# EternityJune25/ComoRAG

Measured on AMD Instinct MI355X. Metric: top-k queries/sec, higher is better.
Workload: dtype bf16; 1 GPU; brute-force top-20 over 10000000 x 768 bf16 rows, batch 64, row-sharded over 1 GPU(s) (north_star target config); rows=10000000, dim=768, batch=64, k=20, query_batches_rotated=4, device=AMD Radeon Graphics (gfx950:sramecc+:xnack-), n_cu=256, repeats=1, exchange=none (1 shard)

## Files before the change

### comorag_amd/csrc/api.hip

```cpp
#include <hip/hip_runtime.h>

#include <algorithm>
#include <cmath>
#include <cstdarg>
#include <cstdio>
#include <cstdlib>
#include <cstring>
#include <chrono>
#include <atomic>
#include <climits>
#include <map>
#include <memory>
#include <mutex>
#include <shared_mutex>
#include <string>
#include <vector>

#include "../../include/comorag_hip.h"
#include "cmr_kernels.h"
#include "cmr_internal.h"
#include "index_state.h"
#include "search_plan.h"
#include "prefilter_host.h"

// ... 30 lines not shown
#define CMR_STR_(x) #x
#define CMR_STR(x) CMR_STR_(x)
#define OPT_FIELD(f) [](cmr_index* i, long long v) { i->f = (decltype(i->f))v; }
#define OPT_READ(expr) [](const cmr_index* i) -> long long { return expr; }
const Option kOptions[] = {
    {"scan_ring", OPT_FIELD(force_ring), Option::any, 0, 0, 0, nullptr, nullptr},
    {"scan_asm_ring", OPT_FIELD(force_asm), Option::any, 0, 0, 0, nullptr, nullptr},
    {"scan_grid", OPT_FIELD(force_grid), Option::any, 0, 0, 0, nullptr, nullptr},
    {"scan_no_sample", OPT_FIELD(no_sample), Option::any, 0, 0, 0, nullptr, nullptr},
    {"scan_no_wide", OPT_FIELD(no_wide), Option::any, 0, 0, 0, nullptr, nullptr},
    {"scan_no_tiny", OPT_FIELD(no_tiny), Option::any, 0, 0, 0, nullptr, nullptr},
    {"scan_no_small", OPT_FIELD(no_small), Option::any, 0, 0, 0, nullptr, nullptr},
    {"small_max_panels", OPT_FIELD(small_max_panels), Option::clamp, 32, 6144, 0, nullptr, nullptr},
    {"tiny_multi", OPT_FIELD(tiny_multi), Option::any, 0, 0, 0, nullptr, nullptr},
    {"zero_copy", OPT_FIELD(zero_copy), Option::any, 0, 0, 0, nullptr, nullptr},
    {"sample_single", OPT_FIELD(single_level), Option::any, 0, 0, 0, nullptr, nullptr},
    {"sample_single_max", OPT_FIELD(single_level_max), Option::clamp, 0, LLONG_MAX, 0, nullptr, nullptr},
    {"sample_tau_in_scan", OPT_FIELD(tau_in_scan), Option::any, 0, 0, 0, nullptr, nullptr},
    {"scan_fin", OPT_FIELD(scan_fin), Option::any, 0, 0, 0, nullptr, nullptr},
    {"sync_poll", OPT_FIELD(sync_poll), Option::any, 0, 0, 0, nullptr, nullptr},
    {"scan_fin_dense", OPT_FIELD(fin_dense), Option::clamp, 1, 1 << 16, 0, nullptr, nullptr},
    {"scan_fin_cap", OPT_FIELD(fin_cap), Option::oneof, 0, 128, 256, "scan_fin_cap must be 0, 128 or 256", nullptr},
    {"scan_fin_suppliers", OPT_FIELD(fin_suppliers), Option::clamp, 0, CMR_FIN_SLOTS / CMR_SCAN_WAVES, 0, nullptr, nullptr},
    {"scan_fin_spin", OPT_FIELD(fin_spin), Option::clamp, 0, 1000, 0, nullptr, nullptr},
    {"scan_fin_queries", OPT_FIELD(fin_max_q), Option::clamp, 1, CMR_FIN_MAX_QUERIES, 0, nullptr, nullptr},
    {"sample_div", OPT_FIELD(sample_div), Option::clamp, 2, LLONG_MAX, 0, nullptr, nullptr},
    {"sample_maxmul", OPT_FIELD(sample_maxmul), Option::clamp, 0, LLONG_MAX, 0, nullptr, nullptr},
    {"pipe_reserve_cus", OPT_FIELD(reserve_cus), Option::any, 0, 0, 0, nullptr, nullptr},
    {"pipe_slots", OPT_FIELD(pipe_slots), Option::any, 0, 0, 0, nullptr, nullptr},
    {"wide_mode", OPT_FIELD(wide_mode), Option::range, 0, 2, 0, "wide_mode must be 0 (default), 1 (register-resident kernel) or 2 (query-split grid)", nullptr},
    {"stream_nt", OPT_FIELD(stream_nt), Option::any, 0, 0, 0, nullptr, nullptr},
    {"pipe_dual_scan", OPT_FIELD(dual_scan), Option::any, 0, 0, 0, nullptr, nullptr},
    {"pipe_cu_mask", OPT_FIELD(cu_mask), Option::any, 0, 0, 0, nullptr, nullptr},
    {"exact_cand", OPT_FIELD(exact_cand), Option::range, 2, CMR_MAX_K, 0, "exact_cand must be in [2, " CMR_STR(CMR_MAX_K) "]", OPT_READ(i->exact_cand)},
    {"combine", [](cmr_index* i, long long v) { i->combine.store((int)v, std::memory_order_relaxed); }, Option::zero_or, 2, cmr_combine::kMaxWidth, 0,
     "combine must be 0 (off) or in [2, " CMR_STR(CMR_PPR_MAX_BATCH) "]", OPT_READ(i->combine.load(std::memory_order_relaxed))},
    {"combine_wait_us", [](cmr_index* i, long long v) { i->combine_wait_us.store(v, std::memory_order_relaxed); }, Option::clamp, 0, 10000000, 0, nullptr,
     OPT_READ(i->combine_wait_us.load(std::memory_order_relaxed))},
    {"prefilter", OPT_FIELD(prefilter), Option::range, -1, 2, 0, "prefilter must be -1 (auto), 0 (off), 1 (on) or 2 (on, the filter keeps every row)", OPT_READ(i->prefilter)},
    {"prefilter_rescore_wgs", OPT_FIELD(pf_rescore_wgs), Option::clamp, 0, 1024, 0, nullptr, nullptr},
    {"prefilter_tighten", OPT_FIELD(pf_tighten), Option::range, 0, 1, 0, "prefilter_tighten must be 0 or 1", OPT_READ(i->pf_tighten)},
    {"prefilter_pair_cap", OPT_FIELD(pf_pair_cap), Option::clamp, 0, 1 << 20, 0, nullptr, OPT_READ(i->pf_pair_cap)},
    {"prefilter_wave_cap", OPT_FIELD(pf_wave_cap), Option::clamp, 0, 1 << 20, 0, nullptr, OPT_READ(i->pf_wave_cap)},
    {"prefilter_sample", OPT_FIELD(pf_sample), Option::range, -1, 1, 0, "prefilter_sample must be -1 (auto), 0 (bf16 sampling) or 1 (int8 sample)", OPT_READ(i->pf_sample)},
    {"prefilter_sample_panels", OPT_FIELD(pf_sample_panels), Option::clamp, 0, INT_MAX, 0, nullptr, OPT_READ(i->pf_sample_panels)},
    {"prefilter_sample_run", OPT_FIELD(pf_sample_run), Option::clamp, 0, 1 << 16, 0, nullptr, OPT_READ(i->pf_sample_run)},
    {"prefilter_sample_wave_cap", OPT_FIELD(pf_sample_wave_cap), Option::clamp, 0, 1 << 20, 0, nullptr, OPT_READ(i->pf_sample_wave_cap)},
    {"prefilter_sample_level0", OPT_FIELD(pf_sample_level0), Option::clamp, 0, 128, 0, nullptr, OPT_READ(i->pf_sample_level0)},
    {"prefilter_sample_active", nullptr, Option::any, 0, 0, 0, nullptr, OPT_READ(i->prefilter_sample_active)},
    {"prefilter_sample_pairs", nullptr, Option::any, 0, 0, 0, nullptr, OPT_READ(q8_read_counter(i, Q8Counter::sample_pairs))},
    {"prefilter_sample_overflow", nullptr, Option::any, 0, 0, 0, nullptr, OPT_READ(q8_read_counter(i, Q8Counter::sample_overflow))},
    {"prefilter_active", nullptr, Option::any, 0, 0, 0, nullptr, OPT_READ(i->prefilter_active)},
    {"prefilter_rows", nullptr, Option::any, 0, 0, 0, nullptr, OPT_READ(i->q8c.q8 ? i->q8c.rows : 0)},
    {"prefilter_bytes", nullptr, Option::any, 0, 0, 0, nullptr, OPT_READ((long long)i->q8c.bytes(i->dpad))},
    {"prefilter_candidates", nullptr, Option::any, 0, 0, 0, nullptr, OPT_READ(q8_read_counter(i, Q8Counter::candidates))},
    {"prefilter_pairs", nullptr, Option::any, 0, 0, 0, nullptr, OPT_READ(q8_read_counter(i, Q8Counter::pairs))},
    {"prefilter_pair_overflow", nullptr, Option::any, 0, 0, 0, nullptr, OPT_READ(q8_read_counter(i, Q8Counter::pair_overflow))},
    {"prefilter_wave_overflow", nullptr, Option::any, 0, 0, 0, nullptr, OPT_READ(q8_read_counter(i, Q8Counter::wave_overflow))},
    {"last_route", nullptr, Option::any, 0, 0, 0, nullptr, OPT_READ(i->last_route.load(std::memory_order_relaxed))},
    {"pipe_dual_scan_active", nullptr, Option::any, 0, 0, 0, nullptr, OPT_READ(i->dual_active)},
    {"pipe_dual_scan_wide_active", nullptr, Option::any, 0, 0, 0, nullptr, OPT_READ(i->dual_wide_active)},
    {"pipe_cu_mask_active", nullptr, Option::any, 0, 0, 0, nullptr, OPT_READ(i->pipe.last_masked)},
    {"pipe_scan_cus", nullptr, Option::any, 0, 0, 0, nullptr, OPT_READ(i->pipe.last_masked ? i->pipe.scan_cus : i->n_cu)},
    {"combine_batches", nullptr, Option::any, 0, 0, 0, nullptr, OPT_READ(i->combiner.batches())},
    {"combine_queries", nullptr, Option::any, 0, 0, 0, nullptr, OPT_READ(i->combiner.queries())},
    {"combine_max_width", nullptr, Option::any, 0, 0, 0, nullptr, OPT_READ(i->combiner.max_width())},
};
#undef OPT_FIELD
#undef OPT_READ

const Option* find_option(const char* name) {
    for (const Option& o : kOptions) if (strcmp(o.name, name) == 0) return &o;
    return nullptr;
}

int set_option(cmr_index* idx, const char* name, long long v) {
    const Option* o = find_option(name ? name : "");
    if (!o || !o->store) return fail(CMR_ERR_INVALID, "unknown option '%s'", name ? name : "");
    const bool refused = o->kind == Option::oneof ? (v != o->a && v != o->b && v != o->c) : o->kind == Option::range ? (v < o->a || v > o->b) : o->kind == Option::zero_or ? (v != 0 && (v < o->a || v > o->b)) : false;
    if (refused) return fail(CMR_ERR_INVALID, "%s", o->reject);
    if (o->kind == Option::clamp) v = std::max(o->a, std::min(v, o->b));
    o->store(idx, v);
    return CMR_OK;
}

int remap_ids_enqueue(cmr_index* idx, int64_t* ids_dev, long long n, hipStream_t s);
long long to_local_row(const cmr_index* idx, long long gid) {
    if (gid < 0) return -1;
    if (idx->single_block()) { const long long r = gid - idx->id_base; return (r >= 0 && r < idx->n) ? r : -1; }
    const size_t nb = idx->blk_local.size();
    size_t b = std::upper_bound(idx->blk_global.begin(), idx->blk_global.end(), gid) - idx->blk_global.begin();
    if (b == 0) return -1;
    --b;
    const long long len = (b + 1 < nb ? idx->blk_local[b + 1] : idx->n) - idx->blk_local[b];
    const long long off = gid - idx->blk_global[b];
    return off < len ? idx->blk_local[b] + off : -1;
// ... 186 lines not shown
        a.fin = (int*)ws->fin_ctl.p; a.fin_pmax = (u64*)ws->fin_pmax.p; a.fin_tau = (u64*)ws->fin_tau.p; a.fin_dense = (u64*)ws->fin_dense.p;
        a.fin_first = p.fin_first; a.fin_wgs = p.fin_wgs; a.fin_mul = p.fin_mul; a.fin_dcap = p.fin_dcap; a.fin_spin = p.fin_spin;
        a.out_ids = ids_dev; a.out_scores = scores_dev; a.out_min = min_dev; a.out_max = max_dev; a.id_base = kernel_id_base(idx);
        fin_state = (const int*)ws->fin_ctl.p + CMR_FIN_STATE;
        if (ws->done_ptr && idx->single_block()) a.fin_done = ws->done_ptr;
    }
    if (p.prefilter) { if ((rc = q8_filter(idx, f, a, sm))) return rc; }
    else HIP_TRY(p.wide ? cmr_launch_scan_wide(g, a, sm) : p.fin ? cmr_launch_scan_fin(g, a, sm) : p.masked ? cmr_launch_scan_masked(g, a, sm) : cmr_launch_scan_topk(g, a, sm));
    if (prof) {
        HIP_TRY(hipEventRecord(pe.b, sm));
        std::lock_guard<std::mutex> pg(idx->prof_mu);
        idx->prof_events.push_back(pe);
        idx->prof_bytes = p.prefilter ? prefilter_bytes(idx, p) : algorithmic_bytes(idx, nqp, k);
    }
    if (a.fin_done) {
        ws->lazy.due = true;
        ws->lazy.lists = (const u64*)ws->lists.p; ws->lazy.cnt = (const int*)ws->cnt.p; ws->lazy.W = p.W; ws->lazy.NQ = p.NQ; ws->lazy.cap = g.cap; ws->lazy.nqp = nqp; ws->lazy.k = k;
        ws->lazy.mm = (const float2*)ws->mm.p; ws->lazy.id_base = kernel_id_base(idx); ws->lazy.ids = ids_dev; ws->lazy.scores = scores_dev; ws->lazy.mn = min_dev; ws->lazy.mx = max_dev;
        ws->lazy.state = fin_state;
        ws->done_used = true;
        return CMR_OK;
    }
    if (sq != sm) {
        HIP_TRY(hipEventRecord(st.ev_scan, sm));
        HIP_TRY(hipStreamWaitEvent(sq, st.ev_scan, 0));
    }
    if (p.prefilter && (rc = q8_rescore(f, sq))) return rc;
    HIP_TRY(cmr_launch_merge_query((const u64*)ws->lists.p, (const int*)ws->cnt.p, p.W, p.NQ, g.cap, nqp, k, (const float2*)ws->mm.p,
                                   kernel_id_base(idx), ids_dev, scores_dev, min_dev, max_dev, nullptr, sq, G > 1, fin_state));
    return remap_ids_enqueue(idx, ids_dev, (long long)nqp * k, sq);
}

int plan_and_enqueue_pass(cmr_index* idx, Workspace* ws, const PassStreams& st, const PassSplit& ps, int k, int reserve_cus, const float* q_dev,
                          const float* min_score, int64_t* ids_dev, float* scores_dev, float* min_dev, float* max_dev, int prefilter = 0) {
    PassPlan plan;
    PassRequest rq = st.request(ps.nqp, k, ps.route, min_score != nullptr, reserve_cus);
    rq.prefilter = prefilter;
    int rc = plan_pass(idx, rq, &plan);
    if (rc) return rc;
    if (ps.q0 == 0)
        idx->last_route.store(route_code(plan, min_score != nullptr) | (ps.nqp < ps.nq ? CMR_ROUTE_MORE_PASSES : 0), std::memory_order_relaxed);
    return enqueue_pass(idx, ws, st, plan, q_dev + (size_t)ps.q0 * idx->dim, min_score, ids_dev + (size_t)ps.q0 * k, scores_dev + (size_t)ps.q0 * k,
                        min_dev ? min_dev + ps.q0 : nullptr, max_dev ? max_dev + ps.q0 : nullptr);
}

int search_enqueue(cmr_index* idx, Workspace* ws, const float* q_dev, int nq, int k, int64_t* ids_dev, float* scores_dev,
                   float* min_dev, float* max_dev, const float* min_score = nullptr) {
    if (k > CMR_MAX_K) {
        if (min_score) return fail(CMR_ERR_UNSUPPORTED, "threshold search supports k <= %d", CMR_MAX_K);
        return search_large_k_enqueue(idx, ws, q_dev, nq, k, ids_dev, scores_dev, min_dev, max_dev);
    }
    if (const int kind = small_path_kind(idx, nq, k, min_score != nullptr)) {
        const long long npanels = idx->npanels();
        idx->last_route.store(route_code(kind == 1 ? CMR_ROUTE_TINY : CMR_ROUTE_SMALL), std::memory_order_relaxed);
        { int rc_ = arm_flag(ws, ws->stream); if (rc_) return rc_; }
        HIP_TRY(ws->d_out.ensure(cmr_tiny_scratch_bytes(nq, (int)npanels, k, idx->tiny_multi, idx->small_max_panels)));
        if (!ws->arrive.p) {
            HIP_TRY(ws->arrive.ensure(sizeof(int)));
            HIP_TRY(hipMemsetAsync(ws->arrive.p, 0, sizeof(int), ws->stream));
        }
        HIP_TRY(cmr_launch_tiny_search(idx->dtype, idx->corpus, q_dev, nq, idx->dim, idx->dpad, idx->n, k, kernel_id_base(idx), ws->d_out.p,
                                       ids_dev, scores_dev, min_dev, max_dev, ws->flag_ptr, idx->tiny_multi ? (int*)ws->arrive.p : nullptr, idx->small_max_panels, ws->stream,
                                       (ws->done_ptr && idx->single_block()) ? ws->done_ptr : nullptr));
        if (ws->done_ptr && idx->single_block()) ws->done_used = true;
        return remap_ids_enqueue(idx, ids_dev, (long long)nq * k, ws->stream);
    }
    const PassStreams st = PassStreams::one(ws->stream);
    for (PassSplit ps(idx, nq); ps.next();) {
        int rc = plan_and_enqueue_pass(idx, ws, st, ps, k, 0, q_dev, min_score, ids_dev, scores_dev, min_dev, max_dev);
        if (rc) return rc;
// ... 59 lines not shown
    Pipe T;
    auto undo = [&]() {
        T.destroy_streams();
        for (auto& slot : ev) for (hipEvent_t& e : slot) if (e) { (void)hipEventDestroy(e); e = nullptr; }
        T.scan_cus = T.wide_cus = 0;
    };
    int rc = create_pipe_streams(idx, T, mask, idx->dual_scan < 0 ? mask != 0 : idx->dual_scan != 0);
    if (rc && mask) {
        undo();
        mask = 0;
        rc = create_pipe_streams(idx, T, 0, idx->dual_scan > 0);
    }
    if (rc) { undo(); return rc; }
    auto make_events = [&]() -> int {
        for (auto& slot : ev) for (hipEvent_t& e : slot) HIP_TRY(hipEventCreateWithFlags(&e, hipEventDisableTiming));
        return CMR_OK;
    };
    rc = make_events();
    if (rc) { undo(); return rc; }
    for (int i = 0; i < Pipe::n_streams; ++i) if (i != Pipe::sq) P.st[i] = T.st[i];
    P.scan_cus = T.scan_cus; P.wide_cus = T.wide_cus;
    for (int i = 0; i < CMR_PIPE_SLOTS; ++i) {
        P.slot[i].pre_done = ev[i][0]; P.slot[i].main_done = ev[i][1]; P.slot[i].scan_done = ev[i][2];
        P.slot[i].ws.stream = P.st[Pipe::sm];
    }
    P.st[Pipe::sq] = T.st[Pipe::sq];
    return CMR_OK;
}

int search_pipelined_enqueue_locked(cmr_index* idx, const float* q_dev, int nq, int k, int64_t* ids_dev, float* scores_dev, float* min_dev,
                                    float* max_dev, hipEvent_t wait_event, hipEvent_t* done_event, const float* min_score, bool may_prefilter = false) {
    Pipe& P = idx->pipe;
    { int rc_ = ensure_pipe(idx); if (rc_) return rc_; }
    P.nslots = std::min(CMR_PIPE_SLOTS, std::max(2, idx->pipe_slots));
    if (k > CMR_MAX_K) return fail(CMR_ERR_UNSUPPORTED, "pipelined search supports k <= %d", CMR_MAX_K);
    const bool masked = P.scan_cus != 0 && (idx->cu_mask > 0 || idx->short_scan());
    const bool twins = P.scan_cus != 0 && !masked;
    P.last_masked = masked ? 1 : 0;
    hipStream_t const nsp = P.st[twins ? Pipe::usp : Pipe::sp], wsp = P.st[twins ? Pipe::uwp : Pipe::wp];
    PassSplit ps(idx, nq);
    if (wait_event) {
        HIP_TRY(hipStreamWaitEvent(nsp, wait_event, 0));
        if (ps.any_wide()) HIP_TRY(hipStreamWaitEvent(wsp, wait_event, 0));
    }
    int prefilter = prefilter_eligible(idx, min_score != nullptr, min_dev || max_dev, nq, may_prefilter);
    if (prefilter && !q8_ensure_companion(idx, nsp)) prefilter = 0;
    idx->prefilter_active = 0;
    idx->prefilter_sample_active = 0;
    PipeSlot* last = nullptr;
    while (ps.next()) {
        const bool wide = ps.wide_streams();
        PipeSlot* sl = &P.slot[P.next++ % (unsigned)P.nslots];
        hipStream_t sp = wide ? wsp : nsp;
        if (sl->used) {
            HIP_TRY(hipStreamWaitEvent(sp, sl->scan_done, 0));
        }
        const bool dual = !twins && P.st[wide ? Pipe::wm2 : Pipe::sm2] != nullptr && (idx->dual_scan > 0 || idx->short_scan());
        if (!wide) idx->dual_active = dual ? 1 : 0;
        else idx->dual_wide_active = dual ? 1 : 0;
        hipStream_t sm = P.st[twins ? (wide ? Pipe::uwm : Pipe::usm)
                                    : wide ? ((dual && (P.nwscan++ & 1)) ? Pipe::wm2 : Pipe::wm) : ((dual && (P.nscan++ & 1)) ? Pipe::sm2 : Pipe::sm)];
        const PassStreams st{sp, sm, P.st[Pipe::sq], sl->pre_done, sl->scan_done, sl->used ? sl->main_done : nullptr};
        int rc = plan_and_enqueue_pass(idx, &sl->ws, st, ps, k, (masked && !wide) ? idx->n_cu - P.scan_cus : (masked && wide) ? idx->n_cu - P.wide_cus : idx->reserve_cus,
                                       q_dev, min_score, ids_dev, scores_dev, min_dev, max_dev, wide ? 0 : prefilter);
        if (rc) return rc;
        HIP_TRY(hipEventRecord(sl->main_done, P.st[Pipe::sq]));
        sl->used = true;
        last = sl;
    }
    if (done_event) *done_event = last ? last->main_done : nullptr;
    return CMR_OK;
}
int search_pipelined_enqueue(cmr_index* idx, const float* q_dev, int nq, int k, int64_t* ids_dev, float* scores_dev, float* min_dev,
                             float* max_dev, hipEvent_t wait_event, hipEvent_t* done_event, const float* min_score = nullptr, bool may_prefilter = false) {
    std::lock_guard<std::mutex> pl(idx->pipe_mu);
    return search_pipelined_enqueue_locked(idx, q_dev, nq, k, ids_dev, scores_dev, min_dev, max_dev, wait_event, done_event, min_score, may_prefilter);
}

int scores_enqueue(cmr_index* idx, Workspace* ws, const float* q_dev, int nq, float* out_dev, long long ld) {
    hipStream_t s = ws->stream;
    CmrScanGeom g{};
    const int per_pass = idx->narrow_width(nq);
    const long long npanels = idx->npanels();
    { int rc_ = arm_flag(ws, s); if (rc_) return rc_; }
    for (int q0 = 0; q0 < nq; q0 += per_pass) {
        const int nqp = std::min(per_pass, nq - q0);
        int rc = make_geom(idx, nqp, 1, false, &g);
        if (rc) return rc;
        HIP_TRY(ws->qfrag.ensure((size_t)g.nqt * g.ks * 1024));
        HIP_TRY(cmr_launch_prep_queries(idx->dtype, q_dev + (size_t)q0 * idx->dim, nqp, idx->dim, idx->dpad, g.nqt, ws->qfrag.p,
                                        ws->flag_ptr, s));
        CmrScanArgs a{};
        a.corpus = idx->corpus; a.qfrag = ws->qfrag.p; a.nrows = idx->n; a.npanels = (int)npanels; a.k = 1;
        a.scores = out_dev + (size_t)q0 * ld; a.ld = ld; a.nq = nqp;
        HIP_TRY(cmr_launch_scan_scores(g, a, s));
    }
    return CMR_OK;
// ... 466 lines not shown
        idx->blk_retired.clear();
    }
    idx->d_blk = d;
    idx->blk_local.assign(local_start, local_start + n_blocks);
    idx->blk_global.assign(global_start, global_start + n_blocks);
    idx->id_base = global_start[0];
    return CMR_OK;
}

int32_t cmr_index_set_option(cmr_index_t* idx, const char* name, int64_t value) {
    if (!idx || !name) return fail(CMR_ERR_INVALID, "NULL argument");
    std::unique_lock<std::shared_mutex> lk(idx->mu);
    return set_option(idx, name, value);
}

int32_t cmr_index_get_option(cmr_index_t* idx, const char* name, int64_t* value) {
    if (!idx || !name || !value) return fail(CMR_ERR_INVALID, "NULL argument");
    std::shared_lock<std::shared_mutex> lk(idx->mu);
    const Option* o = find_option(name);
    if (!o || !o->read) return fail(CMR_ERR_INVALID, "unknown readable option '%s'", name);
    *value = o->read(idx);
    return CMR_OK;
}

int32_t cmr_index_pipeline_stream(cmr_index_t* idx, int32_t which, void** stream) {
    if (!idx || !stream) return fail(CMR_ERR_INVALID, "NULL argument");
    if (which < 0 || which > 2) return fail(CMR_ERR_INVALID, "which must be 0 (pre), 1 (scan) or 2 (post)");
    int rc = cmr_set_device(idx->device);
    if (rc) return rc;
    std::lock_guard<std::mutex> pl(idx->pipe_mu);
    Pipe& P = idx->pipe;
    rc = ensure_pipe(idx);
    if (rc) return rc;
    const bool twins = P.scan_cus != 0 && !P.last_masked && P.next != 0;
    *stream = (void*)P.st[which == 0 ? (twins ? Pipe::usp : Pipe::sp) : which == 1 ? (twins ? Pipe::usm : Pipe::sm) : Pipe::sq];
    return CMR_OK;
}

int32_t cmr_index_query_status(cmr_index_t* idx, int32_t* nonfinite) {
    if (!idx || !nonfinite) return fail(CMR_ERR_INVALID, "NULL argument");
    *nonfinite = 0;
    std::shared_lock<std::shared_mutex> lk(idx->mu);
    int rc = cmr_set_device(idx->device);
    if (rc) return rc;
    std::vector<Workspace*> wss;
    {
        std::lock_guard<std::mutex> pl(idx->pipe_mu);
        for (int i = 0; i < CMR_PIPE_SLOTS; ++i) if (idx->pipe.slot[i].used) wss.push_back(&idx->pipe.slot[i].ws);
        if (idx->pipe.st[Pipe::sq]) {
            for (hipStream_t st : idx->pipe.st) if (st) HIP_TRY(hipStreamSynchronize(st));
        }
    }
    {
        std::lock_guard<std::mutex> g(idx->ws_mu);
        for (auto& kv : idx->stream_ws) wss.push_back(kv.second);
    }
    for (Workspace* ws : wss) {
        if (!ws->flag_ptr) continue;
        if (ws->stream || !ws->own_stream) HIP_TRY(hipStreamSynchronize(ws->stream));
        int h = 0;
        HIP_TRY(hipMemcpy(&h, ws->flag_ptr, sizeof(int), hipMemcpyDeviceToHost));
        if (h) {
            *nonfinite = 1;
            HIP_TRY(hipMemset(ws->flag_ptr, 0, sizeof(int)));
        }
    }
    return CMR_OK;
}
// ... 696 lines not shown
```

### comorag_amd/csrc/index_state.h

```cpp
#pragma once
#include <hip/hip_runtime.h>

#include <algorithm>
#include <atomic>
#include <cstring>
#include <map>
#include <mutex>
#include <shared_mutex>
#include <vector>

#include "../../include/comorag_hip.h"
#include "cmr_kernels.h"
#include "cmr_internal.h"
#include "combine.h"

#define CMR_DT_F32 0
#define CMR_PANEL_ROWS 32
#define CMR_SCAN_WAVES 8
#define CMR_CORPUS_SLACK (128 * 1024)

namespace {

int elem_size(int dtype) { return dtype == CMR_F32 ? 4 : 2; }
int round_up(int x, int m) { return (x + m - 1) / m * m; }
// ... 51 lines not shown
        if (h_pin) { hipError_t e = hipHostFree(h_pin); if (e != hipSuccess) return e; h_pin = nullptr; h_pin_dev = nullptr; h_pin_cap = 0; }
        const size_t want = std::max(need, h_pin_cap * 2);
        hipError_t e = hipHostMalloc(&h_pin, want, hipHostMallocDefault);
        if (e != hipSuccess) return e;
        e = hipHostGetDevicePointer(&h_pin_dev, h_pin, 0);
        if (e != hipSuccess) { (void)hipHostFree(h_pin); h_pin = nullptr; return e; }
        h_pin_cap = want;
        return hipSuccess;
    }
    void release() {
        qfrag.release(); lists.release(); cnt.release(); mm.release(); flag.release(); tau.release();
        s_lists.release(); s_cnt.release(); s_mm.release(); arrive.release();
        fin_ctl.release(); fin_pmax.release(); fin_tau.release(); fin_dense.release(); fin_mm.release();
        d_q.release(); d_ids.release(); d_scores.release(); d_min.release(); d_max.release(); d_cand.release(); d_out.release();
        d_mask.release();
        d_pack.release();
        q8.release();
        x.release();
        if (h_pin) (void)hipHostFree(h_pin);
        h_pin = nullptr; h_pin_dev = nullptr; h_pin_cap = 0;
        if (own_stream && stream) (void)hipStreamDestroy(stream);
    }
};

struct ProfEvent { hipEvent_t a, b; };

constexpr size_t kMappedAppendMax = 128 * 1024;
constexpr size_t kZeroCopyMax = 256 * 1024;

struct PipeSlot { Workspace ws; hipEvent_t pre_done = nullptr, scan_done = nullptr, main_done = nullptr; bool used = false; };
#define CMR_PIPE_SLOTS 4
struct Pipe {
    enum Stream { sp, sm, sm2, wp, wm, wm2, usp, usm, uwp, uwm, sq, n_streams };
    hipStream_t st[n_streams] = {};
    PipeSlot slot[CMR_PIPE_SLOTS]; unsigned next = 0; int nslots = 2; unsigned nscan = 0, nwscan = 0; int scan_cus = 0, wide_cus = 0; int last_masked = 0;
    void destroy_streams() { for (hipStream_t& s : st) if (s) { (void)hipStreamDestroy(s); s = nullptr; } }
};

}

struct cmr_index {
    int device = 0;
    int dim = 0, dpad = 0, dtype = 0;
    uint32_t flags = 0;
    int n_cu = 256;
    long long n = 0;
    long long cap_panels = 0;
    void* corpus = nullptr;
    float* shadow = nullptr;
    std::shared_mutex mu;
    std::mutex ws_mu;
    std::vector<Workspace*> free_ws;
    std::map<hipStream_t, Workspace*> stream_ws;
    DevBuf stage;
    void* h_pin = nullptr;
    void* h_pin_dev = nullptr;
    size_t h_pin_cap = 0;
    int* d_flag = nullptr;
    std::mutex prof_mu;
    bool prof_on = false;
    int prof_every = 1;
    unsigned prof_seq = 0;
    std::vector<ProfEvent> prof_events;
    double prof_bytes = 0.0;
    int force_ring = 0;
    int force_asm = -1;
    int force_grid = 0;
    int no_sample = 0;
// ... 10 lines not shown
    int stream_nt = -1;
    int wide_mode = 0;
    int tau_in_scan = 1;
    int sync_poll = 1;
    int scan_fin = 1;
    int fin_dense = 16384;
    int fin_cap = 0;
    int fin_suppliers = 0;
    int fin_spin = 0;
    int fin_max_q = 8;
    int dual_wide_active = 0;
    std::atomic<long long> last_route{0};
    int dual_active = 0;
    std::atomic<int> combine{0};
    std::atomic<long long> combine_wait_us{0};
    cmr_combine::Combiner combiner;
    long long id_base = 0;
    std::vector<long long> blk_local, blk_global;
    long long* d_blk = nullptr;
    std::vector<void*> blk_retired;
    int sample_maxmul = 0;
    int sample_div = 32;
    int prefilter = -1;
    int pf_rescore_wgs = 0;
    int pf_tighten = 1;
    int pf_pair_cap = 16384;
    int pf_wave_cap = 0;
    int pf_sample = -1;
    int pf_sample_panels = 0;
    int pf_sample_run = 0;
    int pf_sample_wave_cap = 0;
    int pf_sample_level0 = 0;
    int prefilter_sample_active = 0;
    Q8Companion q8c;
    int prefilter_active = 0;
    Q8LastPass q8_last;
    int pipe_slots = 3;
    int reserve_cus = -1;
    std::mutex pipe_mu;
    Pipe pipe;
    float* d_stats = nullptr;
    int exact_cand = CMR_MAX_K;
    ExactScratch x_slot[CMR_PIPE_SLOTS];
    unsigned x_next = 0;

    size_t panel_bytes() const { return (size_t)CMR_PANEL_ROWS * dpad * elem_size(dtype); }
    long long npanels() const { return panels_of(n); }
    int ks() const { return dtype == CMR_F32 ? dpad / 8 : dpad / 16; }
    int narrow_max() const { return cmr_scan_max_nqt(dtype, dpad) >= 2 ? 64 : 32; }
    int narrow_width(int nq) const { return nq > 32 ? narrow_max() : 32; }
    double scan_us() const { return (double)npanels() * panel_bytes() / 6.0e6; }
    bool short_scan() const { return scan_us() < 1000.0; }
    bool single_block() const { return blk_local.size() <= 1; }
    bool small_operands_fit() const { return (size_t)ks() * 1024 <= 143 * 1024; }
};

namespace {

long long kernel_id_base(const cmr_index* idx) { return idx->single_block() ? idx->id_base : 0; }

Workspace* acquire_ws(cmr_index* idx, hipStream_t user_stream, bool dev_api) {
    std::lock_guard<std::mutex> g(idx->ws_mu);
    if (dev_api && user_stream) {
        auto it = idx->stream_ws.find(user_stream);
        if (it != idx->stream_ws.end()) return it->second;
        Workspace* w = new Workspace();
        w->stream = user_stream;
        idx->stream_ws[user_stream] = w;
        return w;
    }
// ... 65 lines not shown
```

### comorag_amd/csrc/search_plan.h

```cpp
#pragma once
#include <numeric>

#include "index_state.h"

bool cmr_ring_audit_ok(int dtype, int nqt, int cap, int ring, int mode);
static const long long kMaxMergeLists = 4096;
constexpr bool kPrefilterSampleAuto = false;
static const long long kQ8SamplePanels = 8192;
static const int kQ8SampleRun = 16;
static const int kQ8SampleLevel0 = 64;

namespace {

int make_geom(const cmr_index* idx, int nq, int k, bool topk, CmrScanGeom* g) {
    const int max_nqt = cmr_scan_max_nqt(idx->dtype, idx->dpad);
    if (max_nqt == 0) return cmr_fail(CMR_ERR_UNSUPPORTED, "dim %d too large for the LDS-resident query tile (dtype %d)", idx->dim, idx->dtype);
    g->dtype = idx->dtype;
    g->dpad = idx->dpad;
    g->nqt = (nq > 32 && max_nqt >= 2) ? 2 : 1;
    g->cap = (topk && k > 32) ? 256 : 128;
    const int ks = idx->ks();
    g->ring = (ks % 16 == 0) ? 16 : 8;
    if (idx->force_ring == 8 || (idx->force_ring == 16 && ks % 16 == 0)) g->ring = idx->force_ring;
    const int mode = topk ? 0 : 1;
    g->asm_ring = cmr_ring_audit_ok(g->dtype, g->nqt, g->cap, g->ring, mode) ? 1 : 0;
    if (idx->force_asm == 0) g->asm_ring = 0;
    if (idx->force_asm == 1 && !cmr_ring_audit_ok(g->dtype, g->nqt, g->cap, g->ring, mode))
        return cmr_fail(CMR_ERR_UNSUPPORTED, "CMR_SCAN_ASM_RING=1 but variant (dtype %d nqt %d cap %d ring %d) failed the ISA audit", g->dtype, g->nqt, g->cap, g->ring);
    if (!cmr_scan_geom(g)) return cmr_fail(CMR_ERR_UNSUPPORTED, "scan geometry does not fit LDS (dpad %d nqt %d)", idx->dpad, g->nqt);
    const int bpc = g->lds <= 80 * 1024 ? 2 : 1;
    long long grid = (idx->npanels() + CMR_SCAN_WAVES - 1) / CMR_SCAN_WAVES;
    grid = std::min<long long>(grid, (long long)idx->n_cu * bpc);
    if (idx->force_grid > 0) grid = std::min<long long>(grid, idx->force_grid);
    g->grid = (int)std::max<long long>(grid, 1);
    return CMR_OK;
}

double algorithmic_bytes(const cmr_index* idx, int nq, int k) {
    return (double)idx->npanels() * CMR_PANEL_ROWS * idx->dpad * elem_size(idx->dtype) + (double)nq * idx->dim * 4 + (double)nq * k * 12;
}

int balanced_grid(long long npanels, int grid, int lists_per_wg) {
    int best = grid;
    double best_cost = -1.0;
    for (int g = grid; g >= std::max(1, grid - grid / 8); --g) {
        const long long W = (long long)g * lists_per_wg;
        const double cost = (double)((npanels + W - 1) / W * W) * (1.0 + 0.0005 * (grid - g));
        if (best_cost < 0 || cost < best_cost) { best_cost = cost; best = g; }
    }
    return best;
}


enum class Route { narrow, wide, quad };

struct PassRequest {
    int nqp = 0, k = 0;
    Route route = Route::narrow;
    bool has_min_score = false;
    bool single_stream = false;
    bool pipelined = false;
    int reserve_cus = 0;
    int prefilter = 0;
    bool masked = false;
};

struct PassPlan {
    int nqp = 0, k = 0;
    bool wide = false;
    CmrScanGeom g{};
    bool fin = false;
    bool masked = false;
    int prefilter = 0;
    int rescore_grid = 0;
    int pair_cap = 0;
    int wave_cap = 0;
    bool sample_q8 = false;
    int s_run = 0, s_stride = 0, s_nruns = 0, s_wave_cap = 0, s_pair_cap = 0;
    int G = 1;
    int n_levels = 0;
    struct Level { long long panels; int grid, Wl, clog, stride; } level[2] = {};
    bool single_level = false;
    bool tau_in_scan = false;
    int reserve_cus = 0;
    int lists_per_wg = CMR_SCAN_WAVES;
    int NQ = 0, W = 0, Ws = 0, tiles = 0, NQA = 0;
    int fin_first = 0, fin_wgs = 0, fin_mul = 1, fin_dcap = 0, fin_spin = 0;
    struct { size_t qfrag, lists, cnt, mm, s_lists, s_cnt, s_mm, tau, fin_ctl, fin_pmax, fin_tau, fin_mm, fin_dense, q8[Q8_NBUF]; } bytes = {};
};

int plan_pass(const cmr_index* idx, const PassRequest& rq, PassPlan* out) {
    PassPlan& p = *out;
    p = PassPlan{};
    const int nqp = rq.nqp, k = rq.k;
    const bool wide = rq.route == Route::wide, quad = rq.route == Route::quad;
    p.nqp = nqp; p.k = k; p.wide = wide;
    if (rq.masked && (wide || quad || rq.prefilter)) return cmr_fail(CMR_ERR_INVALID, "a filtered pass is a narrow pass without the pre-filter");
    p.masked = rq.masked;
    CmrScanGeom& g = p.g;
    const long long npanels = idx->npanels();
    int rc = make_geom(idx, quad ? std::min(nqp, idx->narrow_max()) : nqp, k, true, &g);
    if (rc) return rc;
    const int G = quad ? (nqp + g.nqt * 32 - 1) / (g.nqt * 32) : 1;
    p.G = G;
    g.stream_default_policy = idx->stream_nt < 0 ? (G > 1 ? 1 : 0) : (idx->stream_nt ? 0 : 1);
    const int lists_per_wg = wide ? 1 : CMR_SCAN_WAVES;
// ... 14 lines not shown
    p.fin = fin;
    const bool prefilter = rq.prefilter && !wide && G == 1 && !fin;
    const bool sample_q8 = prefilter && rq.prefilter == 1 && idx->pf_tighten && idx->pf_pair_cap > 0 && npanels >= 4096 &&
                           (idx->pf_sample < 0 ? kPrefilterSampleAuto : idx->pf_sample == 1);
    long long level_panels[2] = {0, 0};
    long long bf16_level1 = 0;
    int n_levels = 0;
    bool single_level = false;
    if (!idx->no_sample && npanels >= 256 && !rq.has_min_score && !fin) {
        const long long s0 = sample_q8 ? std::max<long long>(idx->pf_sample_level0 > 0 ? idx->pf_sample_level0 : kQ8SampleLevel0, k) : std::max<long long>(16, k);
        single_level = !wide && !prefilter && idx->single_level && k <= 32 && nqp <= 8 && npanels >= 4096 && (long long)nqp * npanels <= idx->single_level_max;
        level_panels[n_levels++] = single_level ? 128 : s0;
        if (npanels >= 4096 && !single_level) {
            const long long maxmul = idx->sample_maxmul > 0 ? idx->sample_maxmul : (wide ? 512 : prefilter ? kMaxMergeLists : 128);
            const long long b0 = std::max<long long>(16, k);
            long long s1 = std::min<long long>(std::max<long long>(npanels / idx->sample_div, 8 * b0), maxmul * b0);
            if (!wide) s1 = std::min<long long>(s1, kMaxMergeLists);
            if (s1 < npanels / 2) bf16_level1 = s1;
            if (sample_q8) {
                level_panels[n_levels++] = idx->pf_sample_panels > 0 ? std::min<long long>(idx->pf_sample_panels, npanels)
                                                                     : std::min<long long>(std::max<long long>(npanels / idx->sample_div, 8 * s0), kQ8SamplePanels);
            } else if (bf16_level1) level_panels[n_levels++] = bf16_level1;
        }
    }
    p.n_levels = n_levels;
    p.single_level = single_level;
    p.sample_q8 = sample_q8 && n_levels == 2;
    const long long max_sample = std::max(level_panels[0], p.sample_q8 ? 0 : level_panels[1]);
    int reserve_cus = rq.reserve_cus;
    if (reserve_cus < 0) {
        if (!max_sample) reserve_cus = 0;
        else if (wide) {
            reserve_cus = 32;
        } else if (prefilter && idx->scan_us() >= 1250.0) {
            reserve_cus = 32;
        } else {
            const long long rounds = (long long)((0.7 * idx->scan_us() - 200.0) / 200.0);
            const long long wgs = std::max<long long>(1, (max_sample + lists_per_wg - 1) / lists_per_wg) * G;
            reserve_cus = rounds >= 1 ? (int)std::min<long long>(64, std::max<long long>(8, (wgs + rounds - 1) / rounds)) : 64;
        }
    }
    p.reserve_cus = reserve_cus;
    auto sample_grid = [&](long long spn) -> int {
        if (!wide) return (int)((spn + lists_per_wg - 1) / lists_per_wg);
        const int cap_wgs = rq.pipelined && reserve_cus > 0 ? reserve_cus : idx->n_cu;
        return (int)std::min<long long>(spn, std::max<long long>(cap_wgs, (spn + 47) / 48));
    };
    const int Ws = max_sample ? std::max(sample_grid(level_panels[0]), n_levels > 1 && !p.sample_q8 ? sample_grid(level_panels[1]) : 0) * lists_per_wg : 0;
    int NQ, W, tiles;
    if (wide) {
        const int nqb = cmr_wide_queries(idx->dtype, idx->dpad);
        g.nqt = 1;
        g.grid = (int)std::max<long long>(1, std::min<long long>(npanels, idx->n_cu));
        if (reserve_cus > 0 && g.grid > idx->n_cu / 2) g.grid = std::max(g.grid - reserve_cus, idx->n_cu / 2);
        NQ = nqb; W = g.grid; tiles = nqb / 32;
    } else if (G > 1) {
        if (reserve_cus > 0 && g.grid > idx->n_cu / 2) g.grid = std::max(g.grid - reserve_cus, idx->n_cu / 2);
        int vg = g.grid / G;
        if (vg >= 8) vg &= ~7;
        g.grid = std::max(vg, 1);
        NQ = g.nqt * 32; W = g.grid * CMR_SCAN_WAVES; tiles = G * g.nqt;
    } else {
        if (reserve_cus > 0 && g.grid > idx->n_cu / 2) g.grid = std::max(g.grid - reserve_cus, idx->n_cu / 2);
        if (!idx->force_grid) g.grid = balanced_grid(npanels, g.grid, CMR_SCAN_WAVES);
        NQ = g.nqt * 32; W = g.grid * CMR_SCAN_WAVES; tiles = g.nqt;
    }
    if (prefilter) {
        p.prefilter = rq.prefilter;
        p.rescore_grid = idx->pf_rescore_wgs > 0 ? idx->pf_rescore_wgs : std::min(idx->n_cu, 1024);
        W = p.rescore_grid * cmr_q8_rescore_waves();
        p.pair_cap = (rq.prefilter == 1 && idx->pf_tighten) ? idx->pf_pair_cap : 0;
        p.bytes.q8[Q8_QPACK] = (size_t)2 * tiles * (idx->dpad / 32) * 1024;
        p.bytes.q8[Q8_QCONST] = (size_t)NQ * sizeof(float4);
        p.bytes.q8[Q8_CAND] = (size_t)idx->cap_panels * CMR_PANEL_ROWS * sizeof(unsigned);
        p.bytes.q8[Q8_NCAND] = sizeof(unsigned);
        const long long fw = (long long)g.grid * CMR_SCAN_WAVES;
        p.wave_cap = !p.pair_cap ? 0 : idx->pf_wave_cap > 0 ? idx->pf_wave_cap : (int)std::min<long long>(1 << 20, (((long long)NQ * p.pair_cap + fw - 1) / fw + 63) / 64 * 64);
        p.bytes.q8[Q8_WREC] = std::max<size_t>((size_t)fw * p.wave_cap * 16, 16);
        p.bytes.q8[Q8_WCNT] = (size_t)fw * sizeof(unsigned);
        p.bytes.q8[Q8_PAIR] = std::max<size_t>((size_t)NQ * p.pair_cap * 16, 16);
        p.bytes.q8[Q8_PAIRCNT] = (size_t)NQ * sizeof(unsigned);
        p.bytes.q8[Q8_KEEP] = (size_t)idx->cap_panels * sizeof(unsigned);
        p.bytes.q8[Q8_TAU] = (size_t)NQ * sizeof(float);
        if (p.sample_q8) {
            const long long s1 = level_panels[1];
            const long long run = std::min<long long>(idx->pf_sample_run > 0 ? idx->pf_sample_run : kQ8SampleRun, s1);
            long long nruns = (s1 + run - 1) / run, stride = npanels / nruns;
            if (stride < run) { stride = run; nruns = std::min(nruns, (npanels + run - 1) / run); }
            p.s_run = (int)run; p.s_stride = (int)stride; p.s_nruns = (int)nruns;
            p.s_wave_cap = idx->pf_sample_wave_cap > 0 ? idx->pf_sample_wave_cap : (int)std::min<long long>(1 << 20, (run * CMR_PANEL_ROWS * NQ / 16 + 63) / 64 * 64);
            p.s_pair_cap = p.pair_cap;
            const long long sw = (nruns + CMR_SCAN_WAVES - 1) / CMR_SCAN_WAVES * CMR_SCAN_WAVES;
            p.bytes.q8[Q8_SWREC] = (size_t)sw * p.s_wave_cap * 16;
            p.bytes.q8[Q8_SWCNT] = (size_t)sw * sizeof(unsigned);
            p.bytes.q8[Q8_SPAIR] = (size_t)NQ * p.s_pair_cap * 16;
            p.bytes.q8[Q8_SPAIRCNT] = (size_t)NQ * sizeof(unsigned);
        }
    }
    const int NQA = G * NQ;
    p.NQ = NQ; p.W = W; p.Ws = Ws; p.tiles = tiles; p.NQA = NQA;
    p.bytes.qfrag = (size_t)tiles * g.ks * 1024;
// ... 14 lines not shown
        }
        L.grid = sample_grid(spn);
        L.Wl = L.grid * lists_per_wg;
        L.grid *= G;
        L.clog = spn >= 64 ? 3 : 0;
        const long long nchunks = (spn + (1 << L.clog) - 1) >> L.clog;
        L.stride = (int)(npanels / nchunks);
    }
    p.tau_in_scan = n_levels > 0 && single_level && idx->tau_in_scan && NQ == 32 && nqp <= 2 && k <= 64 && !p.prefilter;
    if (G > 1) g.grid *= G;
    if (fin) {
        p.fin_dcap = idx->fin_dense;
        p.fin_spin = idx->fin_spin;
        p.bytes.fin_ctl = CMR_FIN_CTL * sizeof(int);
        p.bytes.fin_pmax = (size_t)32 * CMR_FIN_SLOTS * 8;
        p.bytes.fin_tau = 32 * 8;
        p.bytes.fin_mm = (size_t)32 * 512 * 8;
        p.bytes.fin_dense = (size_t)32 * p.fin_dcap * 8;
        p.fin_first = std::min(g.grid, idx->n_cu);
        p.fin_wgs = std::min(std::min(idx->fin_suppliers > 0 ? idx->fin_suppliers : (npanels >= 131072 ? 128 : 64), CMR_FIN_SLOTS / CMR_SCAN_WAVES), p.fin_first);
        p.fin_mul = 1;
        for (int m = std::max(1, (int)(g.grid * 0.6180339887)); m < g.grid; ++m)
            if (std::gcd(m, g.grid) == 1) { p.fin_mul = m; break; }
    }
    return CMR_OK;
}

long long route_code(int path, int n_levels = 0, bool tau_in_scan = false, bool single_level = false, int nqt = 1, bool threshold = false) {
    return (long long)path | ((long long)n_levels << 4) | ((long long)(tau_in_scan ? 1 : 0) << 6) | ((long long)(single_level ? 1 : 0) << 7) | ((long long)nqt << 8) |
           ((long long)(threshold ? 1 : 0) << 10);
}
long long route_code(const PassPlan& p, bool threshold) {
    const int path = p.wide ? CMR_ROUTE_WIDE : p.G > 1 ? CMR_ROUTE_QUERY_SPLIT : p.fin ? CMR_ROUTE_FIN : CMR_ROUTE_CHAIN;
    return route_code(path, p.n_levels, p.tau_in_scan, p.single_level, p.g.nqt, threshold) | (p.masked ? CMR_ROUTE_FILTERED : 0);
}


bool wide_pass_is_quad(const cmr_index* idx) {
    if (idx->wide_mode == 2) return true;
    if (idx->wide_mode == 1) return false;
    return cmr_wide_queries(idx->dtype, idx->dpad) == 0;
}
bool short_two_tile_pass(const cmr_index* idx, int left) {
    if (idx->wide_mode != 0 || idx->no_wide || cmr_wide_queries(idx->dtype, idx->dpad) == 0) return false;
    if (cmr_scan_max_nqt(idx->dtype, idx->dpad) < 2 || left <= 64 || left > 128) return false;
    return idx->short_scan();
}
int wide_pass_queries(const cmr_index* idx) {
    if (idx->no_wide) return 0;
    if (!wide_pass_is_quad(idx)) return cmr_wide_queries(idx->dtype, idx->dpad);
    return 4 * idx->narrow_max();
}

struct PassSplit {
    const cmr_index* idx;
    const int nq, narrow, wideq;
    const bool quad;
    int q0 = 0, nqp = 0;
    Route route = Route::narrow;
    PassSplit(const cmr_index* i, int nq_) : idx(i), nq(nq_), narrow(i->narrow_width(nq_)), wideq(wide_pass_queries(i)), quad(wide_pass_is_quad(i)) {}
    bool any_wide() const { return wideq > 0 && nq > narrow; }
    bool wide_streams() const { return route != Route::narrow; }
    bool next() {
        q0 += nqp;
        if (q0 >= nq) return false;
        const int left = nq - q0;
        const bool wide = wideq > 0 && left > narrow;
// ... 16 lines not shown
```

### include/comorag_hip.h

```cpp
#ifndef COMORAG_HIP_H
#define COMORAG_HIP_H

#include <stdint.h>

#ifdef __cplusplus
extern "C" {
#endif

#define CMR_ABI_VERSION 2

enum cmr_status {
    CMR_OK = 0,
    CMR_ERR_INVALID = -1,
    CMR_ERR_NO_DEVICE = -2,
    CMR_ERR_HIP = -3,
    CMR_ERR_OOM = -4,
    CMR_ERR_NONFINITE = -5,
    CMR_ERR_UNSUPPORTED = -6
};

enum cmr_dtype { CMR_F32 = 0, CMR_BF16 = 1, CMR_F16 = 2 };

#define CMR_FLAG_KEEP_F32 1u

// ... 17 lines not shown

int32_t cmr_index_append(cmr_index_t* idx, const float* rows_f32, int64_t n);
int32_t cmr_index_append_dev(cmr_index_t* idx, const float* rows_f32_dev, int64_t n, void* stream);

int32_t cmr_index_search(cmr_index_t* idx, const float* q_f32, int32_t nq, int32_t k,
                         int64_t* out_ids, float* out_scores, float* out_min, float* out_max);
int32_t cmr_index_search_min_score(cmr_index_t* idx, const float* q_f32, int32_t nq, int32_t k, float min_score,
                                   int64_t* out_ids, float* out_scores);
int32_t cmr_index_search_min_score_dev(cmr_index_t* idx, const float* q_f32_dev, int32_t nq, int32_t k, float min_score,
                                       int64_t* out_ids_dev, float* out_scores_dev, void* stream);
int32_t cmr_index_search_min_score_pipelined(cmr_index_t* idx, const float* q_f32_dev, int32_t nq, int32_t k, float min_score,
                                             int64_t* out_ids_dev, float* out_scores_dev, void* wait_event, void** done_event);
int32_t cmr_index_search_dev(cmr_index_t* idx, const float* q_f32_dev, int32_t nq, int32_t k,
                             int64_t* out_ids_dev, float* out_scores_dev, float* out_min_dev,
                             float* out_max_dev, void* stream);

int32_t cmr_index_search_masked(cmr_index_t* idx, const float* q_f32, int32_t nq, int32_t k,
                                const uint32_t* allow_words, int64_t n_words,
                                int64_t* out_ids, float* out_scores, float* out_min, float* out_max);
int32_t cmr_index_search_masked_dev(cmr_index_t* idx, const float* q_f32_dev, int32_t nq, int32_t k,
                                    const uint32_t* allow_words_dev, int64_t n_words,
                                    int64_t* out_ids_dev, float* out_scores_dev,
                                    float* out_min_dev, float* out_max_dev, void* stream);

int32_t cmr_index_search_pipelined(cmr_index_t* idx, const float* q_f32_dev, int32_t nq, int32_t k,
                                   int64_t* out_ids_dev, float* out_scores_dev, float* out_min_dev,
                                   float* out_max_dev, void* wait_event, void** done_event);

int32_t cmr_index_set_id_base(cmr_index_t* idx, int64_t base);
int32_t cmr_index_set_id_blocks(cmr_index_t* idx, int32_t n_blocks, const int64_t* local_start, const int64_t* global_start);
int32_t cmr_index_set_option(cmr_index_t* idx, const char* name, int64_t value);
#define CMR_ROUTE_MORE_PASSES (1 << 11)
#define CMR_ROUTE_FILTERED (1 << 12)
#define CMR_ROUTE_TINY 1
#define CMR_ROUTE_SMALL 2
#define CMR_ROUTE_CHAIN 3
#define CMR_ROUTE_FIN 4
#define CMR_ROUTE_WIDE 5
#define CMR_ROUTE_QUERY_SPLIT 6
#define CMR_ROUTE_LARGE_K 7
#define CMR_ROUTE_SCORES_SINGLE 8
#define CMR_ROUTE_SCORES 9
#define CMR_ROUTE_SORTED 10
int32_t cmr_index_get_option(cmr_index_t* idx, const char* name, int64_t* value);
int32_t cmr_index_pipeline_stream(cmr_index_t* idx, int32_t which, void** stream);

int32_t cmr_index_query_status(cmr_index_t* idx, int32_t* nonfinite);

int32_t cmr_stream_wait_event(void* stream, void* event);
int32_t cmr_event_synchronize(void* event);

int32_t cmr_index_scores(cmr_index_t* idx, const float* q_f32, int32_t nq, float* out, int64_t ld);
int32_t cmr_index_scores_dev(cmr_index_t* idx, const float* q_f32_dev, int32_t nq, float* out_dev,
                             int64_t ld, void* stream);

int32_t cmr_index_sorted_scores(cmr_index_t* idx, const float* q_f32, int32_t nq, int64_t* out_ids,
                                float* out_scores, float* out_min, float* out_max);

int32_t cmr_index_rescore(cmr_index_t* idx, const float* q_f32, int32_t nq, const int64_t* cand,
                          int32_t n_cand, int32_t k, int64_t* out_ids, float* out_scores);

int32_t cmr_index_search_exact(cmr_index_t* idx, const float* q_f32, int32_t nq, int32_t k, int64_t* out_ids, float* out_scores,
                               int32_t* out_exact);
int32_t cmr_index_search_exact_pipelined(cmr_index_t* idx, const float* q_f32_dev, int32_t nq, int32_t k, int64_t* ids_dev,
                                         float* scores_dev, int32_t* exact_dev, void* wait_event, void** done_event);
int32_t cmr_index_round_stats(cmr_index_t* idx, float* max_row_norm, float* max_round_err);
// ... 136 lines not shown
```

Baseline: 41760 queries/s.

## Route prefiltered narrow passes onto CU-masked wide stream set with dual scan streams

Adds a 'filter' pipeline stream set that sends prefiltered narrow passes through the CU-masked wide-stream pair (wp/wm/wm2). On long scans it can alternate between two scan streams, reserving the non-wide CUs for the prefilter and rescore work. The set is picked automatically when the prefilter is active, the scan is long and the batch is wider than 32 queries. Slot count becomes set-dependent: 2 for the filter set and 3 otherwise. This aims to overlap prefilter and scan stages better, at the cost of fewer slots and a different CU partition.

```diff
diff --git a/comorag_amd/csrc/api.hip b/comorag_amd/csrc/api.hip
--- a/comorag_amd/csrc/api.hip
+++ b/comorag_amd/csrc/api.hip
@@ -86,6 +86,8 @@
     {"stream_nt", OPT_FIELD(stream_nt), Option::any, 0, 0, 0, nullptr, nullptr},
     {"pipe_dual_scan", OPT_FIELD(dual_scan), Option::any, 0, 0, 0, nullptr, nullptr},
     {"pipe_cu_mask", OPT_FIELD(cu_mask), Option::any, 0, 0, 0, nullptr, nullptr},
+    {"pipe_prefilter_dual", OPT_FIELD(pf_dual), Option::range, -1, 1, 0, "pipe_prefilter_dual must be -1 (auto), 0 (off) or 1 (on)", OPT_READ(i->pf_dual)},
+    {"pipe_prefilter_dual_active", nullptr, Option::any, 0, 0, 0, nullptr, OPT_READ(i->pf_dual_active)},
     {"exact_cand", OPT_FIELD(exact_cand), Option::range, 2, CMR_MAX_K, 0, "exact_cand must be in [2, " CMR_STR(CMR_MAX_K) "]", OPT_READ(i->exact_cand)},
     {"combine", [](cmr_index* i, long long v) { i->combine.store((int)v, std::memory_order_relaxed); }, Option::zero_or, 2, cmr_combine::kMaxWidth, 0,
      "combine must be 0 (off) or in [2, " CMR_STR(CMR_PPR_MAX_BATCH) "]", OPT_READ(i->combine.load(std::memory_order_relaxed))},
@@ -115,7 +117,7 @@
     {"pipe_dual_scan_active", nullptr, Option::any, 0, 0, 0, nullptr, OPT_READ(i->dual_active)},
     {"pipe_dual_scan_wide_active", nullptr, Option::any, 0, 0, 0, nullptr, OPT_READ(i->dual_wide_active)},
     {"pipe_cu_mask_active", nullptr, Option::any, 0, 0, 0, nullptr, OPT_READ(i->pipe.last_masked)},
-    {"pipe_scan_cus", nullptr, Option::any, 0, 0, 0, nullptr, OPT_READ(i->pipe.last_masked ? i->pipe.scan_cus : i->n_cu)},
+    {"pipe_scan_cus", nullptr, Option::any, 0, 0, 0, nullptr, OPT_READ(i->pipe.last_masked ? i->pipe.last_scan_cus : i->n_cu)},
     {"combine_batches", nullptr, Option::any, 0, 0, 0, nullptr, OPT_READ(i->combiner.batches())},
     {"combine_queries", nullptr, Option::any, 0, 0, 0, nullptr, OPT_READ(i->combiner.queries())},
     {"combine_max_width", nullptr, Option::any, 0, 0, 0, nullptr, OPT_READ(i->combiner.max_width())},
@@ -368,10 +370,11 @@
 }
 
 int plan_and_enqueue_pass(cmr_index* idx, Workspace* ws, const PassStreams& st, const PassSplit& ps, int k, int reserve_cus, const float* q_dev,
-                          const float* min_score, int64_t* ids_dev, float* scores_dev, float* min_dev, float* max_dev, int prefilter = 0) {
+                          const float* min_score, int64_t* ids_dev, float* scores_dev, float* min_dev, float* max_dev, int prefilter = 0, bool filter_set = false) {
     PassPlan plan;
     PassRequest rq = st.request(ps.nqp, k, ps.route, min_score != nullptr, reserve_cus);
     rq.prefilter = prefilter;
+    rq.filter_set = filter_set;
     int rc = plan_pass(idx, rq, &plan);
     if (rc) return rc;
     if (ps.q0 == 0)
@@ -497,19 +500,32 @@
                                     float* max_dev, hipEvent_t wait_event, hipEvent_t* done_event, const float* min_score, bool may_prefilter = false) {
     Pipe& P = idx->pipe;
     { int rc_ = ensure_pipe(idx); if (rc_) return rc_; }
-    P.nslots = std::min(CMR_PIPE_SLOTS, std::max(2, idx->pipe_slots));
     if (k > CMR_MAX_K) return fail(CMR_ERR_UNSUPPORTED, "pipelined search supports k <= %d", CMR_MAX_K);
     const bool masked = P.scan_cus != 0 && (idx->cu_mask > 0 || idx->short_scan());
     const bool twins = P.scan_cus != 0 && !masked;
-    P.last_masked = masked ? 1 : 0;
-    hipStream_t const nsp = P.st[twins ? Pipe::usp : Pipe::sp], wsp = P.st[twins ? Pipe::uwp : Pipe::wp];
+    int prefilter = prefilter_eligible(idx, min_score != nullptr, min_dev || max_dev, nq, may_prefilter);
+    int set = pipe_stream_set(idx, prefilter, nq, P.scan_cus, P.wide_cus, P.st[Pipe::wm2] != nullptr);
+    hipStream_t nsp = P.st[Pipe::pre_of(set)];
+    hipStream_t const wsp = P.st[twins ? Pipe::uwp : Pipe::wp];
     PassSplit ps(idx, nq);
     if (wait_event) {
         HIP_TRY(hipStreamWaitEvent(nsp, wait_event, 0));
         if (ps.any_wide()) HIP_TRY(hipStreamWaitEvent(wsp, wait_event, 0));
     }
-    int prefilter = prefilter_eligible(idx, min_score != nullptr, min_dev || max_dev, nq, may_prefilter);
-    if (prefilter && !q8_ensure_companion(idx, nsp)) prefilter = 0;
+    if (prefilter && !q8_ensure_companion(idx, nsp)) {
+        prefilter = 0;
+        if (set == Pipe::set_filter) {
+            set = pipe_stream_set(idx, 0, nq, P.scan_cus, P.wide_cus, false);
+            nsp = P.st[Pipe::pre_of(set)];
+            if (wait_event) HIP_TRY(hipStreamWaitEvent(nsp, wait_event, 0));
+        }
+    }
+    const bool fset = set == Pipe::set_filter;
+    P.nslots = pipe_slot_count(idx, set);
+    P.last_set = set;
+    P.last_masked = masked || fset ? 1 : 0;
+    P.last_scan_cus = fset ? P.wide_cus : P.scan_cus;
+    idx->pf_dual_active = 0;
     idx->prefilter_active = 0;
     idx->prefilter_sample_active = 0;
     PipeSlot* last = nullptr;
@@ -520,14 +536,18 @@
         if (sl->used) {
             HIP_TRY(hipStreamWaitEvent(sp, sl->scan_done, 0));
         }
-        const bool dual = !twins && P.st[wide ? Pipe::wm2 : Pipe::sm2] != nullptr && (idx->dual_scan > 0 || idx->short_scan());
+        const bool fpass = fset && !wide;
+        const bool dual = fpass ? idx->dual_scan != 0 : (!twins && P.st[wide ? Pipe::wm2 : Pipe::sm2] != nullptr && (idx->dual_scan > 0 || idx->short_scan()));
         if (!wide) idx->dual_active = dual ? 1 : 0;
         else idx->dual_wide_active = dual ? 1 : 0;
-        hipStream_t sm = P.st[twins ? (wide ? Pipe::uwm : Pipe::usm)
-                                    : wide ? ((dual && (P.nwscan++ & 1)) ? Pipe::wm2 : Pipe::wm) : ((dual && (P.nscan++ & 1)) ? Pipe::sm2 : Pipe::sm)];
+        if (fpass) idx->pf_dual_active = 1;
+        hipStream_t sm = P.st[fpass ? ((dual && (P.nwscan++ & 1)) ? Pipe::wm2 : Pipe::wm)
+                              : twins ? (wide ? Pipe::uwm : Pipe::usm)
+                                      : wide ? ((dual && (P.nwscan++ & 1)) ? Pipe::wm2 : Pipe::wm) : ((dual && (P.nscan++ & 1)) ? Pipe::sm2 : Pipe::sm)];
         const PassStreams st{sp, sm, P.st[Pipe::sq], sl->pre_done, sl->scan_done, sl->used ? sl->main_done : nullptr};
-        int rc = plan_and_enqueue_pass(idx, &sl->ws, st, ps, k, (masked && !wide) ? idx->n_cu - P.scan_cus : (masked && wide) ? idx->n_cu - P.wide_cus : idx->reserve_cus,
-                                       q_dev, min_score, ids_dev, scores_dev, min_dev, max_dev, wide ? 0 : prefilter);
+        int rc = plan_and_enqueue_pass(idx, &sl->ws, st, ps, k,
+                                       fpass ? idx->n_cu - P.wide_cus : (masked && !wide) ? idx->n_cu - P.scan_cus : (masked && wide) ? idx->n_cu - P.wide_cus : idx->reserve_cus,
+                                       q_dev, min_score, ids_dev, scores_dev, min_dev, max_dev, wide ? 0 : prefilter, fpass);
         if (rc) return rc;
         HIP_TRY(hipEventRecord(sl->main_done, P.st[Pipe::sq]));
         sl->used = true;
@@ -1060,8 +1080,8 @@
     Pipe& P = idx->pipe;
     rc = ensure_pipe(idx);
     if (rc) return rc;
-    const bool twins = P.scan_cus != 0 && !P.last_masked && P.next != 0;
-    *stream = (void*)P.st[which == 0 ? (twins ? Pipe::usp : Pipe::sp) : which == 1 ? (twins ? Pipe::usm : Pipe::sm) : Pipe::sq];
+    const int set = P.next != 0 ? P.last_set : Pipe::set_base;
+    *stream = (void*)P.st[which == 0 ? Pipe::pre_of(set) : which == 1 ? Pipe::scan_of(set) : Pipe::sq];
     return CMR_OK;
 }
 
diff --git a/comorag_amd/csrc/index_state.h b/comorag_amd/csrc/index_state.h
--- a/comorag_amd/csrc/index_state.h
+++ b/comorag_amd/csrc/index_state.h
@@ -107,8 +107,13 @@
 #define CMR_PIPE_SLOTS 4
 struct Pipe {
     enum Stream { sp, sm, sm2, wp, wm, wm2, usp, usm, uwp, uwm, sq, n_streams };
+    enum Set { set_base, set_twins, set_filter };
     hipStream_t st[n_streams] = {};
     PipeSlot slot[CMR_PIPE_SLOTS]; unsigned next = 0; int nslots = 2; unsigned nscan = 0, nwscan = 0; int scan_cus = 0, wide_cus = 0; int last_masked = 0;
+    int last_set = set_base;
+    int last_scan_cus = 0;
+    static Stream pre_of(int set) { return set == set_twins ? usp : set == set_filter ? wp : sp; }
+    static Stream scan_of(int set) { return set == set_twins ? usm : set == set_filter ? wm : sm; }
     void destroy_streams() { for (hipStream_t& s : st) if (s) { (void)hipStreamDestroy(s); s = nullptr; } }
 };
 
@@ -185,10 +190,12 @@
     int pf_sample_wave_cap = 0;
     int pf_sample_level0 = 0;
     int prefilter_sample_active = 0;
+    int pf_dual = -1;
+    int pf_dual_active = 0;
     Q8Companion q8c;
     int prefilter_active = 0;
     Q8LastPass q8_last;
-    int pipe_slots = 3;
+    int pipe_slots = 0;
     int reserve_cus = -1;
     std::mutex pipe_mu;
     Pipe pipe;
diff --git a/comorag_amd/csrc/search_plan.h b/comorag_amd/csrc/search_plan.h
--- a/comorag_amd/csrc/search_plan.h
+++ b/comorag_amd/csrc/search_plan.h
@@ -51,6 +51,23 @@
     return best;
 }
 
+bool prefilter_long_scan(const cmr_index* idx) { return idx->scan_us() >= 1250.0; }
+
+constexpr bool kPrefilterDualAuto = true;
+int pipe_stream_set(const cmr_index* idx, int prefilter, int nq, int scan_cus, int wide_cus, bool second_filter_stream) {
+    const bool masked = scan_cus != 0 && (idx->cu_mask > 0 || idx->short_scan());
+    if (prefilter && wide_cus != 0 && second_filter_stream && idx->pf_dual != 0) {
+        if (idx->pf_dual > 0) return Pipe::set_filter;
+        if (kPrefilterDualAuto && idx->cu_mask < 0 && idx->reserve_cus < 0 && prefilter_long_scan(idx) && idx->narrow_width(nq) > 32) return Pipe::set_filter;
+    }
+    return masked || scan_cus == 0 ? Pipe::set_base : Pipe::set_twins;
+}
+
+int pipe_slot_count(const cmr_index* idx, int set) {
+    if (idx->pipe_slots <= 0) return set == Pipe::set_filter ? 2 : 3;
+    return std::min(CMR_PIPE_SLOTS, std::max(2, idx->pipe_slots));
+}
+
 
 enum class Route { narrow, wide, quad };
 
@@ -63,6 +80,7 @@
     int reserve_cus = 0;
     int prefilter = 0;
     bool masked = false;
+    bool filter_set = false;
 };
 
 struct PassPlan {
@@ -72,6 +90,7 @@
     bool fin = false;
     bool masked = false;
     int prefilter = 0;
+    bool filter_set = false;
     int rescore_grid = 0;
     int pair_cap = 0;
     int wave_cap = 0;
@@ -152,7 +171,7 @@
         if (!max_sample) reserve_cus = 0;
         else if (wide) {
             reserve_cus = 32;
-        } else if (prefilter && idx->scan_us() >= 1250.0) {
+        } else if (prefilter && prefilter_long_scan(idx)) {
             reserve_cus = 32;
         } else {
             const long long rounds = (long long)((0.7 * idx->scan_us() - 200.0) / 200.0);
@@ -187,6 +206,7 @@
     }
     if (prefilter) {
         p.prefilter = rq.prefilter;
+        p.filter_set = rq.filter_set;
         p.rescore_grid = idx->pf_rescore_wgs > 0 ? idx->pf_rescore_wgs : std::min(idx->n_cu, 1024);
         W = p.rescore_grid * cmr_q8_rescore_waves();
         p.pair_cap = (rq.prefilter == 1 && idx->pf_tighten) ? idx->pf_pair_cap : 0;
@@ -267,7 +287,7 @@
 }
 long long route_code(const PassPlan& p, bool threshold) {
     const int path = p.wide ? CMR_ROUTE_WIDE : p.G > 1 ? CMR_ROUTE_QUERY_SPLIT : p.fin ? CMR_ROUTE_FIN : CMR_ROUTE_CHAIN;
-    return route_code(path, p.n_levels, p.tau_in_scan, p.single_level, p.g.nqt, threshold) | (p.masked ? CMR_ROUTE_FILTERED : 0);
+    return route_code(path, p.n_levels, p.tau_in_scan, p.single_level, p.g.nqt, threshold) | (p.masked ? CMR_ROUTE_FILTERED : 0) | (p.filter_set ? CMR_ROUTE_PREFILTER_DUAL : 0);
 }
 
 
diff --git a/include/comorag_hip.h b/include/comorag_hip.h
--- a/include/comorag_hip.h
+++ b/include/comorag_hip.h
@@ -73,6 +73,7 @@
 int32_t cmr_index_set_option(cmr_index_t* idx, const char* name, int64_t value);
 #define CMR_ROUTE_MORE_PASSES (1 << 11)
 #define CMR_ROUTE_FILTERED (1 << 12)
+#define CMR_ROUTE_PREFILTER_DUAL (1 << 13)
 #define CMR_ROUTE_TINY 1
 #define CMR_ROUTE_SMALL 2
 #define CMR_ROUTE_CHAIN 3
```

Result: faster. 43400 queries/s, median of 6 (+3.9%).
